# tensorboy/centerpose

Hardware: AMD Instinct MI355X
Metric: images/sec end-to-end (backbone+decode), DLA-34 512x512 (higher is better)
Workload: dtype f32

## Files before the change

centerpose_amd/csrc/plan_runtime.cpp:

```cpp
#include <cstdio>
#include <cstring>
#include <memory>
#include <string>
#include <vector>
#include "common.h"

extern "C" {
struct cp_conv_desc;
struct cp_dcn_desc;
int cp_abi_version(void);
int cp_conv2d_f32(const cp_conv_desc*, const float* const*, const float*, const float*, const float*, const float*, float*, void*);
int cp_conv3x3_winograd_f32(const cp_conv_desc*, const float*, const float*, const float*, const float*, const float*, float*, void*);
int cp_dcn_v2_f32(const cp_dcn_desc*, const float*, const float*, const float*, const float*, const float*, float*, void*);
int cp_conv3x3_winograd24_group_f32(const cp_conv_desc*, int, const float* const*, const float* const*, const float* const*, const float* const*,
                                    const float* const*, float* const*, void*);
int cp_conv2d_group_f32(const cp_conv_desc*, int, const float* const*, const float* const*, const float* const*, const float* const*,
                        const float* const*, float* const*, void*);
int cp_stem7x7_f32(const float*, const float*, const float*, const float*, float*, int, int, int, int, int, int, int, void*);
int cp_maxpool2d_nhwc_f32(const float*, int, float*, int, int, int, int, int, int, int, int, void*);
int cp_dw_deconv_add_nhwc_f32(const float*, int, const float*, const float*, int, float*, int, int, int, int, int, int, void*);
int cp_sum_up_nhwc_f32(int, const float* const*, const int*, const int*, float*, int, int, int, int, int, int, void*);
int cp_sum_up_group_nhwc_f32(int, const float* const*, const int*, float* const*, int, void*);
int cp_head3x3_1x1_f32(const cp_conv_desc*, const float*, const float*, const float*, const float*, const float*, const float*, float*, int,
                       int, int, void*);
int cp_dwconv2d_nhwc_f32(const float*, int, const float*, const float*, const float*, float*, int, int, int, int, int, int, int, int, int, void*);
int cp_global_avgpool_nhwc_f32(const float*, int, float*, int, int, int, int, void*);
int cp_scale_add_nhwc_f32(const float*, int, const float*, int, const float*, int, float*, int, int, int, int, int, void*);
int cp_shuffle_concat_nhwc_f32(const float*, int, const float*, int, float*, int, long long, int, int, void*);
int cp_multi_pose_decode_f32(const float*, const float*, const float*, const float*, const float*, const float*, int, int, int, int,
                             int, int, float*, float*, int*, void*);
int cp_splitk_reduce_f32(const float*, int, int, int, const float*, const float*, int, float*, int, int, void*);
int cp_sizeof_conv_desc(void);
int cp_sizeof_dcn_desc(void);
int cp_decode_topk_f32(const float*, const float*, int, int, int, int, int, int, float*, int*, void*);
int cp_decode_assign_f32(const float*, const float*, const float*, const float*, const float*, const int*, int, int, int, int, int, float*,
                         void*);
int cp_head_points_f32(const float*, int, const int*, const float*, const float*, const float*, const float*, float*, int, int, int, int, int,
                       int, int, void*);
int cp_flip_merge_pairs_f32(int, const float* const*, float* const*, const int*, int, int, int, int, const int*, void*);
int cp_head_points_pairs_f32(const float*, int, const int*, const int*, const float*, const float*, const float*, const float*, float*, int, int,
                             int, int, int, int, int, void*);
}

namespace {

enum { FN_CONV = 1, FN_WINO = 2, FN_DCN = 3, FN_STEM7 = 4, FN_POOL = 5, FN_UPADD = 6, FN_SUMUP = 7, FN_DWCONV = 8, FN_AVGPOOL = 9,
       FN_SCALEADD = 10, FN_SHUFFLE = 11, FN_HEAD = 12, FN_TOPK = 13, FN_ASSIGN = 14, FN_SPLITK = 15, FN_WINO24G = 16, FN_CONVG = 17, FN_SUMUPG = 18,
       FN_POINTS = 19, FN_FLIPPAIRS = 20, FN_POINTSPAIRS = 21 };
enum { REF_NULL = 0, REF_BUF = 1, REF_CONST = 2 };

struct Op {
    uint32_t fn = 0, out_index = 0, stream = 0;
    std::vector<unsigned char> desc;
    std::vector<float*> ptrs;
    std::vector<int> bufid;
    std::vector<int> ints;
};

struct Out { float* p; int shape[4]; int bufid; };

struct ConstPool {
    std::vector<float*> p;
    ~ConstPool() { for (float* q : p) if (q) (void)hipFree(q); }
};

}

struct cp_plan {
    int B = 0, H = 0, W = 0;
    std::vector<float*> bufs;
    std::vector<uint64_t> buf_numel;
// ... 36 lines not shown
    const int* I = o.ints.data();
    switch (o.fn) {
        case FN_CONV:
            return cp_conv2d_f32(reinterpret_cast<const cp_conv_desc*>(o.desc.data()), reinterpret_cast<const float* const*>(P.data()), P[4],
                                 P[5], P[6], P[7], P[8], s);
        case FN_WINO:
            return cp_conv3x3_winograd_f32(reinterpret_cast<const cp_conv_desc*>(o.desc.data()), P[0], P[1], P[2], P[3], P[4], P[5], s);
        case FN_DCN:
            return cp_dcn_v2_f32(reinterpret_cast<const cp_dcn_desc*>(o.desc.data()), P[0], P[1], P[2], P[3], P[4], P[5], s);
        case FN_WINO24G:
            return cp_conv3x3_winograd24_group_f32(reinterpret_cast<const cp_conv_desc*>(o.desc.data()), I[0], reinterpret_cast<const float* const*>(P.data()),
                                                   reinterpret_cast<const float* const*>(P.data() + 4), reinterpret_cast<const float* const*>(P.data() + 8),
                                                   reinterpret_cast<const float* const*>(P.data() + 12), reinterpret_cast<const float* const*>(P.data() + 16),
                                                   reinterpret_cast<float* const*>(P.data() + 20), s);
        case FN_CONVG:
            return cp_conv2d_group_f32(reinterpret_cast<const cp_conv_desc*>(o.desc.data()), I[0], reinterpret_cast<const float* const*>(P.data()),
                                       reinterpret_cast<const float* const*>(P.data() + 8), reinterpret_cast<const float* const*>(P.data() + 16),
                                       reinterpret_cast<const float* const*>(P.data() + 24), reinterpret_cast<const float* const*>(P.data() + 32),
                                       reinterpret_cast<float* const*>(P.data() + 40), s);
        case FN_STEM7:
            return cp_stem7x7_f32(P[0], P[1], P[2], P[3], P[4], I[0], I[1], I[2], I[3], I[4], I[5], I[6], s);
        case FN_POOL:
            return cp_maxpool2d_nhwc_f32(P[0], I[0], P[1], I[1], I[2], I[3], I[4], I[5], I[6], I[7], I[8], s);
        case FN_UPADD:
            return cp_dw_deconv_add_nhwc_f32(P[0], I[0], P[1], P[2], I[1], P[3], I[2], I[3], I[4], I[5], I[6], I[7], s);
        case FN_SUMUP:
            return cp_sum_up_nhwc_f32(I[0], reinterpret_cast<const float* const*>(P.data()), I + 1, I + 5, P[4], I[9], I[10], I[11], I[12],
                                      I[13], I[14], s);
        case FN_SUMUPG:
            return cp_sum_up_group_nhwc_f32(I[0], reinterpret_cast<const float* const*>(P.data()), I + 2, reinterpret_cast<float* const*>(P.data() + 16), I[1], s);
        case FN_HEAD:
            return cp_head3x3_1x1_f32(reinterpret_cast<const cp_conv_desc*>(o.desc.data()), P[0], P[1], P[2], P[3], P[4], P[5], P[6], I[0], I[1],
                                      I[2], s);
        case FN_DWCONV:
            return cp_dwconv2d_nhwc_f32(P[0], I[0], P[1], P[2], P[3], P[4], I[1], I[2], I[3], I[4], I[5], I[6], I[7], I[8], I[9], s);
        case FN_AVGPOOL:
            return cp_global_avgpool_nhwc_f32(P[0], I[0], P[1], I[1], I[2], I[3], I[4], s);
        case FN_SCALEADD:
            return cp_scale_add_nhwc_f32(P[0], I[0], P[1], I[1], P[2], I[2], P[3], I[3], I[4], I[5], I[6], I[7], s);
        case FN_SHUFFLE:
            return cp_shuffle_concat_nhwc_f32(P[0], I[0], P[1], I[1], P[2], I[2], (long long)I[3], I[4], I[5], s);
        case FN_SPLITK:
            return cp_splitk_reduce_f32(P[0], I[0], I[1], I[2], P[1], P[2], I[3], P[3], I[4], I[5], s);
        case FN_TOPK:
            return cp_decode_topk_f32(P[0], P[1], I[0], I[1], I[2], I[3], I[4], I[5], P[2], reinterpret_cast<int*>(P[3]), s);
        case FN_ASSIGN:
// ... 2 lines not shown
            return cp_head_points_f32(P[0], I[0], reinterpret_cast<const int*>(P[1]), P[2], P[3], P[4], P[5], P[6], I[1], I[2], I[3], I[4], I[5],
                                      I[6], I[7], s);
        case FN_FLIPPAIRS:
            return cp_flip_merge_pairs_f32(I[0], reinterpret_cast<const float* const*>(P.data()), reinterpret_cast<float* const*>(P.data() + 4), I + 5,
                                           I[1], I[2], I[3], I[4], reinterpret_cast<const int*>(P[8]), s);
        case FN_POINTSPAIRS:
            return cp_head_points_pairs_f32(P[0], I[0], reinterpret_cast<const int*>(P[1]), reinterpret_cast<const int*>(P[2]), P[3], P[4], P[5],
                                            P[6], P[7], I[1], I[2], I[3], I[4], I[5], I[6], I[7], s);
    }
    cp_set_error("plan: unknown launch function %u", o.fn);
    return 1;
}

bool arity_ok(const Op& o)
{
    switch (o.fn) {
        case FN_CONV: return o.ptrs.size() == 9 && (int)o.desc.size() == cp_sizeof_conv_desc();
        case FN_WINO: return o.ptrs.size() == 6 && (int)o.desc.size() == cp_sizeof_conv_desc();
        case FN_DCN: return o.ptrs.size() == 6 && (int)o.desc.size() == cp_sizeof_dcn_desc();
        case FN_WINO24G: return o.ptrs.size() == 25 && o.ints.size() == 1 && o.ints[0] >= 1 && o.ints[0] <= 4 && (int)o.desc.size() == 4 * cp_sizeof_conv_desc();
        case FN_CONVG: return o.ptrs.size() == 49 && o.ints.size() == 1 && o.ints[0] >= 1 && o.ints[0] <= 8 && (int)o.desc.size() == 8 * cp_sizeof_conv_desc();
        case FN_STEM7: return o.ptrs.size() == 5 && o.ints.size() == 7;
        case FN_POOL: return o.ptrs.size() == 2 && o.ints.size() == 9;
        case FN_UPADD: return o.ptrs.size() == 4 && o.ints.size() == 8;
        case FN_SUMUP: return o.ptrs.size() == 5 && o.ints.size() == 15;
        case FN_SUMUPG: return o.ptrs.size() == 21 && o.ints.size() == 58 && o.ints[0] >= 1 && o.ints[0] <= 4;
        case FN_HEAD: return o.ptrs.size() == 7 && o.ints.size() == 3 && (int)o.desc.size() == cp_sizeof_conv_desc();
        case FN_DWCONV: return o.ptrs.size() == 5 && o.ints.size() == 10;
        case FN_AVGPOOL: return o.ptrs.size() == 2 && o.ints.size() == 5;
        case FN_SCALEADD: return o.ptrs.size() == 4 && o.ints.size() == 8;
        case FN_SHUFFLE: return o.ptrs.size() == 3 && o.ints.size() == 6;
        case FN_SPLITK: return o.ptrs.size() == 4 && o.ints.size() == 6;
        case FN_TOPK: return o.ptrs.size() == 4 && o.ints.size() == 6;
        case FN_ASSIGN: return o.ptrs.size() == 7 && o.ints.size() == 5;
        case FN_POINTS: return o.ptrs.size() == 7 && o.ints.size() == 8;
        case FN_FLIPPAIRS: return o.ptrs.size() == 10 && o.ints.size() == 13 && o.ints[0] >= 1 && o.ints[0] <= 4;
        case FN_POINTSPAIRS: return o.ptrs.size() == 8 && o.ints.size() == 8;
    }
    return false;
}

int run_all(cp_plan* pl, hipStream_t s)
{
    for (const Op& o : pl->ops)
        if (int rc = run_op(o, s)) return rc;
    return 0;
// ... 440 lines not shown
```

centerpose_amd/engine.py:

```python
import os
import warnings
import weakref

import torch

from . import _lib, nets, ops
from .nets import Act


DECODE_TOPK = "decode.nms_topk"
SPARSE_HEADS = ("wh", "hps", "reg", "hp_offset")
FLIP_PEAKS = "flip.merge_peaks"
FLIP_IDX = ((1, 2), (3, 4), (5, 6), (7, 8), (9, 10), (11, 12), (13, 14), (15, 16))


def normalize_state_dict(sd, arch=None):
    out = {}
    for k, v in sd.items():
        if k.startswith("module") and not k.startswith("module_list"):
            k = k[7:]
        out[nets.internal_key(arch, k) if arch is not None else k] = v
    return out


# ... 23 lines not shown

    def give(self, slot):
        if self.reuse:
            self.free.append((self.clock(), slot))


class PlanBuilder(nets.Graph):
    def __init__(self, sd, B, device, sigmoid_heads=True, const_cache=None, dets_only=False):
        super().__init__()
        self.dets_only = dets_only
        self.points = None
        self.sd, self.B, self.dev = sd, B, device
        self.const_cache = const_cache if const_cache is not None else {}
        self.pool = BufferPool(device, lambda: len(self.launches))
        if isinstance(sigmoid_heads, bool):
            sigmoid_heads = ("hm", "hm_hp") if sigmoid_heads else ()
        self.sigmoid_heads = tuple(sigmoid_heads)
        self.launches = []
        self.winograd = os.environ.get("CP_WINOGRAD", "1") != "0"
        self.dcn_splitk = os.environ.get("CP_DCN_SPLITK", "1") != "0"
        self.wino_splitc = os.environ.get("CP_WINO_SPLITC", "1") != "0"
        self.conv_splitk = os.environ.get("CP_CONV_SPLITK", "1") != "0"
        self.fuse_heads = os.environ.get("CP_FUSE_HEADS", "1") != "0"
        self._pool_cache = {}
        self.outputs = None

    @property
    def bytes_alloc(self):
        return self.pool.bytes

    def buf(self, H, W, C, split=None):
        Cp = 2 * split[1] if split else ops.round_up(C, 16)
        slot = self.pool.take(self.B * H * W * Cp)
        act = Act(H, W, C, slot[: self.B * H * W * Cp].view(self.B, H, W, Cp), split)
        weakref.finalize(act, self.pool.give, slot)
        return act

    @staticmethod
    def cmap(a):
        if a.split:
            h, hp = a.split
            return list(range(h)) + list(range(hp, hp + h))
        return list(range(a.C))

    def expand_in(self, w, xs):
        if all(a.t.shape[3] == a.C and not a.split for a in xs):
            return w
# ... 54 lines not shown
        self.pool.give(ws)

    def add_conv3x3(self, name, flops, x, wp, u, sc, sh, out, cout, act, res=None, splitc=True):
        kind, wu = u if u is not None else ("conv", None)
        kw = dict(kh=3, kw=3, stride=1, pad=1, cout=cout, wino=wu, tile=ops.WINO24 if kind == "wino24" else 0)
        B, H, W, cin = x.shape
        S = ops.wino_ksplit(B, H, W, cin, cout) if (splitc and kind == "wino" and self.wino_splitc and res is None) else 1
        if S > 1:
            self.add_split(kind, name, ".splitc", flops, S, B * H * W, out.shape[3], lambda ones, zeros, ws: ops.conv2d_launch(
                [x], wp, ones, zeros, ws, ksplit=S, **kw), sc, sh, out, cout, act)
        else:
            self.add(kind, name, flops, ops.conv2d_launch([x], wp, sc, sh, out, act=act, res=res, **kw))

    def group_bufs(self, shapes):
        sizes = [self.B * H * W * Cp for H, W, _, Cp in shapes]
        slot = self.pool.take(sum(sizes))
        holder = Act(1, 1, 1, slot)
        weakref.finalize(holder, self.pool.give, slot)
        whole = slot[:sum(sizes)]
        return [Act(H, W, C, v.view(self.B, H, W, Cp), parent=holder) for (H, W, C, Cp), v in zip(shapes, whole.split(sizes))], whole

    def emit_conv(self, xs, conv, bn, bias, co, k, stride, pad, relu, res, stem):
        x = xs[0]
        Ho, Wo = (x.H + 2 * pad - k) // stride + 1, (x.W + 2 * pad - k) // stride + 1
        out = self.buf(Ho, Wo, co)
        if stem and k == 7 and pad == 3 and co in (16, 64) and res is None and bn and relu in (True, False):
            wp7 = ops.pack_stem7_weight(self.w(conv + ".weight"))
            sc7, sh7 = ops.fold_bn(co, self.bn(bn), self.w(conv + ".bias") if bias else None, self.dev)
            self.add("conv", conv, 2 * Ho * Wo * co * 3 * 49, ops.stem7x7_launch(xs[0].t, wp7, sc7, sh7, out.t, stride, relu))
            return out
        w = self.w(conv + ".weight")
        wp = ops.pack_conv_weight(w if stem else self.expand_in(w, xs), stem=stem)
        sc, sh = ops.fold_bn(co, self.bn(bn) if bn else None, self.w(conv + ".bias") if bias else None, self.dev)
        srcs = [a.t for a in xs]
        rt = res.t if res is not None else None
        ci = sum(a.C for a in xs)
        cip = ci if stem else sum(a.t.shape[3] for a in xs)
        u = None if stem else self.wino(wp, cip, co, conv, k, stride, pad, len(xs), hw=(x.H, x.W))
        flops = 2 * Ho * Wo * co * ci * k * k
        S = ops.conv_ksplit(ops.rule_batch(self.B) * Ho * Wo, wp.shape[0], wp.shape[1]) \
            if (self.conv_splitk and not stem and len(xs) == 1 and res is None and not (k == 3 and stride == 1 and pad == 1)) else 1
        if u is not None:
            self.add_conv3x3(conv, flops, srcs[0], wp, u, sc, sh, out.t, out.t.shape[3], self.act_code(relu), rt)
        elif S > 1:
            self.add_split("conv", conv, ".splitk", flops, S, self.B * Ho * Wo, wp.shape[0], lambda ones, zeros, ws: ops.conv2d_launch(
                srcs, wp, ones, zeros, ws, kh=k, kw=k, stride=stride, pad=pad, cout=ws.shape[2], ksplit=S),
# ... 31 lines not shown
            chunk = members[c0:c0 + ops.GROUP_MAX]
            if len(chunk) == 1:
                outs += super().emit_conv_batch(chunk)
                continue
            couts, whole = self.group_bufs([((x.H + 2 * pad - k) // stride + 1, (x.W + 2 * pad - k) // stride + 1, co, ops.round_up(co, 16))
                                            for x, _, _, co, k, stride, pad, _ in chunk])
            recs, flops = [], 0
            for (x, conv, bn, co, k, stride, pad, relu), out in zip(chunk, couts):
                wp = ops.pack_conv_weight(self.expand_in(self.w(conv + ".weight"), [x]))
                sc, sh = ops.fold_bn(co, self.bn(bn), None, self.dev)
                ldw = ops.round_up(wp.shape[0], 64)
                recs.append(dict(x=x.t, wp=ops.pad_rows(wp, ldw), scale=ops.pad_vec(sc, ldw), shift=ops.pad_vec(sh, ldw), out=out.t,
                                 cout=out.t.shape[3], k=k, stride=stride, pad=pad, act=self.act_code(relu)))
                flops += 2 * out.H * out.W * co * x.C * k * k
            self.add("conv", "group:" + chunk[0][1], flops, ops.conv2d_group_launch(recs, whole))
            outs += couts
        return outs

    def emit_maxpool(self, x, k, s, p):
        key = (id(x), k, s, p)
        hit = self._pool_cache.get(key)
        if hit is not None and hit[0]() is x and hit[1]() is not None:
            return hit[1]()
        out = self.buf((x.H + 2 * p - k) // s + 1, (x.W + 2 * p - k) // s + 1, x.C)
        self.add("pool", "maxpool%dx%d" % (k, k), 0, ops.maxpool2d_launch(x.t, out.t, k, s, p))
        self._pool_cache[key] = (weakref.ref(x), weakref.ref(out))
        return out

    def emit_dcn(self, x, conv, bn, co):
        om = self.buf(x.H, x.W, 32)
        wom = ops.pack_conv_weight(self.expand_in(self.w(conv + ".conv_offset_mask.weight"), [x]))
        som, hom = ops.fold_bn(27, None, self.w(conv + ".conv_offset_mask.bias"), self.dev)
        som[27:] = 0.0
        out = self.buf(x.H, x.W, co)
        wp = ops.pack_conv_weight(self.expand_in(self.w(conv + ".weight"), [x]))
        sc, sh = ops.fold_bn(co, self.bn(bn), self.w(conv + ".bias"), self.dev)
        uom = self.wino(wom, x.t.shape[3], 32, conv + ".conv_offset_mask", hw=(x.H, x.W))
        self.add_conv3x3(conv + ".conv_offset_mask", 2 * x.H * x.W * 27 * x.C * 9, x.t, wom, uom, som, hom, om.t, 32, ops.ACT_NONE)
        flops = 2 * x.H * x.W * co * x.C * 9
        S = ops.dcn_ksplit(ops.rule_batch(self.B) * x.H * x.W, wp.shape[0]) if self.dcn_splitk else 1
        if S > 1:
            self.add_split("dcn", conv, ".splitk", flops, S, self.B * x.H * x.W, wp.shape[0], lambda ones, zeros, ws: ops.dcn_v2_launch(
                x.t, om.t, wp, ones, zeros, ws, cout=ws.shape[2], om_sigmoid=True, ksplit=S), sc, sh, out.t, out.t.shape[3], ops.ACT_RELU)
        else:
            self.add("dcn", conv, flops,
                     ops.dcn_v2_launch(x.t, om.t, wp, sc, sh, out.t, cout=out.t.shape[3], om_sigmoid=True, act=ops.ACT_RELU))
        return out

    def emit_up_add(self, x, wname, f, add):
        out = self.buf(x.H * f, x.W * f, x.C)
# ... 439 lines not shown
        if g is None:
            g = torch.cuda.CUDAGraph()
            with torch.cuda.graph(g, capture_error_mode="thread_local"):
                self.run_eager()
            self.stream_of_launch = [0] * len(self.launches)
        self.graph = g

    def forward(self, images):
        if tuple(images.shape) != tuple(self.input.shape):
            raise ValueError("engine was planned for input %s, got %s" % (tuple(self.input.shape), tuple(images.shape)))
        if images.data_ptr() != self.input.data_ptr():
            self.input.copy_(images)
        if self.use_graph:
            if self.graph is None:
                self.capture()
            self.graph.replay()
        else:
            self.run_eager()
        return self.outputs

    __call__ = forward

    def launch_bytes(self, launches=None):
        grouped = ("cp_conv3x3_winograd24_group_f32", "cp_conv2d_group_f32", "cp_sum_up_group_nhwc_f32", "cp_flip_merge_pairs_f32")
        return [sum(4 * t.numel() for t in (launch.tensors[:-1] if launch.fn in grouped else launch.tensors) if t is not None)
                for _, _, _, launch in (self.launches if launches is None else launches)]

    def profile(self, iters=5):
        torch.cuda.synchronize(self.device)
        self.run_eager()
        nbytes = self.launch_bytes()
        recs = []
        for (kind, name, flops, launch), nb in zip(self.launches, nbytes):
            e0, e1 = torch.cuda.Event(enable_timing=True), torch.cuda.Event(enable_timing=True)
            e0.record()
            for _ in range(iters):
                launch.run()
            e1.record()
            e1.synchronize()
            recs.append(dict(kind=kind, name=name, fn=launch.fn, kernel=launch.kernel, flops=flops, bytes=nb, ms=e0.elapsed_time(e1) / iters))
        return recs

    def profile_in_sequence(self, iters=10):
        torch.cuda.synchronize(self.device)
        self.run_eager()
        n = len(self.launches)
        samples = [[] for _ in range(n)]
# ... 69 lines not shown
```

centerpose_amd/nets.py:

```python
from collections import OrderedDict

HEADS = (("hm", 1), ("wh", 2), ("hps", 34), ("reg", 2), ("hm_hp", 17), ("hp_offset", 2))
ARCH_HEAD = {"dla_34": (64, 256), "res_50": (256, 64), "hrnet": (32, 64), "mobilenetv3": (24, 256), "shufflenetV2": (256, 256),
             "resdcn_18": (64, 64), "resdcn_34": (64, 64), "resdcn_50": (64, 64), "resdcn_101": (64, 64)}
RESDCN_SPEC = {18: ("basic", [2, 2, 2, 2]), 34: ("basic", [3, 4, 6, 3]), 50: ("bottleneck", [3, 4, 6, 3]),
               101: ("bottleneck", [3, 4, 23, 3])}


class Act:
    __slots__ = ("H", "W", "C", "t", "split", "parent", "__weakref__")

    def __init__(self, H, W, C, t=None, split=None, parent=None):
        self.H, self.W, self.C, self.t, self.split = H, W, C, t, split
        self.parent = parent


class Graph:

    def __init__(self):
        self.spec = OrderedDict()
        self.flops = 0

    def p_conv(self, name, co, ci, k, bias=False, kw=None):
        self.spec[name + ".weight"] = (co, ci, k, kw or k)
        if bias:
            self.spec[name + ".bias"] = (co,)

    def p_bn(self, name, c):
        for s in ("weight", "bias", "running_mean", "running_var"):
            self.spec["%s.%s" % (name, s)] = (c,)
        self.spec[name + ".num_batches_tracked"] = ()

    def emit_conv(self, xs, conv, bn, bias, co, k, stride, pad, relu, res, stem):
        x = xs[0]
        return Act((x.H + 2 * pad - k) // stride + 1, (x.W + 2 * pad - k) // stride + 1, co)

    def emit_maxpool(self, x, k, s, p):
        return Act((x.H + 2 * p - k) // s + 1, (x.W + 2 * p - k) // s + 1, x.C)

    def emit_conv_group(self, members):
        return [self.emit_conv([x], conv, bn, False, co, 3, 1, 1, relu, res, False) for x, conv, bn, co, relu, res in members]

    def emit_conv_batch(self, members):
        return [self.emit_conv([x], conv, bn, False, co, k, stride, pad, relu, None, False) for x, conv, bn, co, k, stride, pad, relu in members]

    def emit_dcn(self, x, conv, bn, co):
        return Act(x.H, x.W, co)

    def emit_up_add(self, x, wname, f, add):
        return Act(x.H * f, x.W * f, x.C)

    def emit_deconv4(self, x, wname, bn, co):
        return Act(x.H * 2, x.W * 2, co)

    def emit_sum_up(self, xs, shifts, relu):
        return Act(xs[0].H, xs[0].W, xs[0].C)

    def emit_sum_up_batch(self, members, relu):
        return [self.emit_sum_up(xs, shifts, relu) for xs, shifts in members]

    def emit_head(self, feat, p, hc):
# ... 38 lines not shown
    def dwconv(self, x, name, bn, k, stride, act=None):
        self.spec[name + ".weight"] = (x.C, 1, k, k)
        self.p_bn(bn, x.C)
        out = self.emit_dwconv(x, name, bn, k, stride, act)
        self.flops += 2 * out.H * out.W * x.C * k * k
        return out

    def up_add(self, x, wname, f, add):
        self.spec[wname + ".weight"] = (x.C, 1, 2 * f, 2 * f)
        out = self.emit_up_add(x, wname, f, add)
        self.flops += 2 * out.H * out.W * x.C * 4
        return out

    def _dla_block(self, x, p, ci, co, stride, residual):
        h = self.conv(x, p + ".conv1", p + ".bn1", co, 3, stride, 1, relu=True)
        return self.conv(h, p + ".conv2", p + ".bn2", co, 3, 1, 1, relu=True, res=residual)

    def _dla_tree(self, x, p, levels, ci, co, stride, level_root, root_dim=0, children=None, top=True):
        children = [] if children is None else children
        if root_dim == 0:
            root_dim = 2 * co
        if level_root:
            root_dim += ci
        bottom = self.emit_maxpool(x, stride, stride, 0) if stride > 1 else x
        if ci != co:
            self.p_conv(p + ".project.0", co, ci, 1)
            self.p_bn(p + ".project.1", co)
        if level_root:
            children.append(bottom)
        if levels == 1:
            residual = bottom
            if ci != co:
                residual = self.emit_conv([bottom], p + ".project.0", p + ".project.1", False, co, 1, 1, 0, False, None, False)
                self.flops += 2 * residual.H * residual.W * co * ci
            x1 = self._dla_block(x, p + ".tree1", ci, co, stride, residual)
            x2 = self._dla_block(x1, p + ".tree2", co, co, 1, x1)
            return self.conv([x2, x1] + children, p + ".root.conv", p + ".root.bn", co, 1, relu=True)
        x1 = self._dla_tree(x, p + ".tree1", levels - 1, ci, co, stride, False)
        children.append(x1)
        return self._dla_tree(x1, p + ".tree2", levels - 1, co, co, 1, False, root_dim + co, children)

    def dla34(self, x, p="backbone_model"):
        ch, lv = [16, 32, 64, 128, 256, 512], [1, 1, 1, 2, 2, 1]
        b = p + ".base"
        y = []
        x = self.conv(x, b + ".base_layer.0", b + ".base_layer.1", 16, 7, 1, 3, relu=True, stem=True)
        x = self.conv(x, b + ".level0.0", b + ".level0.1", 16, 3, 1, 1, relu=True)
# ... 283 lines not shown
```

centerpose_amd/ops.py:

```python
import ctypes
import os

import torch

from . import _lib

ACT_NONE, ACT_RELU, ACT_SIGMOID, ACT_HSWISH, ACT_HSIGMOID = 0, 1, 2, 3, 4
BN_EPS = 1e-5


class ConvDesc(ctypes.Structure):
    _fields_ = [(n, ctypes.c_int) for n in ("nsrc",)] + [("srcC", ctypes.c_int * 4), ("srcLd", ctypes.c_int * 4)] + \
        [(n, ctypes.c_int) for n in ("B", "H", "W", "Ho", "Wo", "kh", "kw", "sy", "sx", "py", "px", "K", "ldw", "Cout",
                                     "resLd", "outLd", "outNCHW", "OH", "OW", "osy", "osx", "ooy", "oox", "act",
                                     "inNCHW", "tile", "nsub", "ksplit")]


class DcnDesc(ctypes.Structure):
    _fields_ = [(n, ctypes.c_int) for n in ("B", "H", "W", "C", "srcLd", "Ho", "Wo", "kh", "kw", "sy", "sx", "py", "px",
                                            "dily", "dilx", "K", "ldw", "Cout", "omLd", "omSigmoid", "outLd",
                                            "outNCHW", "act", "tile", "ksplit", "dg")]


def round_up(x, m):
# ... 31 lines not shown
        if self.kernel is None:
            self.kernel = _lib.lib().cp_last_kernel().decode()


def marshal(fn, desc, ptrs, ints):
    d = ctypes.byref(desc) if desc is not None else None
    if fn == "cp_conv2d_f32":
        srcs = (ctypes.c_void_p * 4)(*[p.value for p in ptrs[:4]])
        return [d, srcs] + ptrs[4:]
    if fn in ("cp_conv3x3_winograd_f32", "cp_dcn_v2_f32"):
        return [d] + ptrs
    if fn == "cp_conv3x3_winograd24_group_f32":
        arr = lambda k: (ctypes.c_void_p * 4)(*[p.value for p in ptrs[4 * k:4 * k + 4]])
        return [d, ints[0]] + [arr(k) for k in range(6)]
    if fn == "cp_conv2d_group_f32":
        arr = lambda k: (ctypes.c_void_p * 8)(*[p.value for p in ptrs[8 * k:8 * k + 8]])
        return [d, ints[0]] + [arr(k) for k in range(6)]
    if fn == "cp_head3x3_1x1_f32":
        return [d] + ptrs + ints
    if fn == "cp_stem7x7_f32":
        return ptrs + ints
    if fn == "cp_maxpool2d_nhwc_f32":
        return [ptrs[0], ints[0], ptrs[1]] + ints[1:]
    if fn == "cp_dw_deconv_add_nhwc_f32":
        return [ptrs[0], ints[0], ptrs[1], ptrs[2], ints[1], ptrs[3]] + ints[2:]
    if fn == "cp_sum_up_nhwc_f32":
        srcs = (ctypes.c_void_p * 4)(*[p.value for p in ptrs[:4]])
        lds = (ctypes.c_int * 4)(*ints[1:5])
        shs = (ctypes.c_int * 4)(*ints[5:9])
        return [ints[0], srcs, lds, shs, ptrs[4]] + ints[9:]
    if fn == "cp_sum_up_group_nhwc_f32":
        srcs = (ctypes.c_void_p * 16)(*[p.value for p in ptrs[:16]])
        outs = (ctypes.c_void_p * 4)(*[p.value for p in ptrs[16:20]])
        meta = (ctypes.c_int * 56)(*ints[2:58])
        return [ints[0], srcs, meta, outs, ints[1]]
    if fn == "cp_dwconv2d_nhwc_f32":
        return [ptrs[0], ints[0], ptrs[1], ptrs[2], ptrs[3], ptrs[4]] + ints[1:]
    if fn == "cp_global_avgpool_nhwc_f32":
        return [ptrs[0], ints[0], ptrs[1]] + ints[1:]
    if fn == "cp_scale_add_nhwc_f32":
        return [ptrs[0], ints[0], ptrs[1], ints[1], ptrs[2], ints[2], ptrs[3]] + ints[3:]
    if fn == "cp_shuffle_concat_nhwc_f32":
        return [ptrs[0], ints[0], ptrs[1], ints[1], ptrs[2], ints[2], ctypes.c_longlong(ints[3]), ints[4], ints[5]]
    if fn == "cp_splitk_reduce_f32":
        return [ptrs[0], ints[0], ints[1], ints[2], ptrs[1], ptrs[2], ints[3], ptrs[3], ints[4], ints[5]]
    if fn == "cp_decode_topk_f32":
        return ptrs[:2] + ints + ptrs[2:]
    if fn == "cp_decode_assign_f32":
        return ptrs[:6] + ints + [ptrs[6]]
    if fn == "cp_head_points_f32":
        return [ptrs[0], ints[0]] + ptrs[1:] + ints[1:]
    if fn == "cp_head_points_pairs_f32":
        return [ptrs[0], ints[0]] + ptrs[1:] + ints[1:]
    if fn == "cp_flip_merge_pairs_f32":
        ins = (ctypes.c_void_p * 4)(*[p.value for p in ptrs[:4]])
        outs = (ctypes.c_void_p * 4)(*[p.value for p in ptrs[4:8]])
        meta = (ctypes.c_int * 8)(*ints[5:13])
        return [ints[0], ins, outs, meta] + ints[1:5] + [ptrs[8]]
    raise ValueError("unknown launch function %r" % fn)


FN_IDS = {"cp_conv2d_f32": 1, "cp_conv3x3_winograd_f32": 2, "cp_dcn_v2_f32": 3, "cp_stem7x7_f32": 4,
          "cp_maxpool2d_nhwc_f32": 5, "cp_dw_deconv_add_nhwc_f32": 6, "cp_sum_up_nhwc_f32": 7, "cp_dwconv2d_nhwc_f32": 8,
          "cp_global_avgpool_nhwc_f32": 9, "cp_scale_add_nhwc_f32": 10, "cp_shuffle_concat_nhwc_f32": 11, "cp_head3x3_1x1_f32": 12,
          "cp_decode_topk_f32": 13, "cp_decode_assign_f32": 14, "cp_splitk_reduce_f32": 15, "cp_conv3x3_winograd24_group_f32": 16, "cp_conv2d_group_f32": 17,
          "cp_sum_up_group_nhwc_f32": 18, "cp_head_points_f32": 19,
          "cp_flip_merge_pairs_f32": 20, "cp_head_points_pairs_f32": 21}


def pad_rows(t, ldw):
    Co, K = t.shape
    if Co == ldw:
        return t.contiguous()
    out = torch.zeros((ldw, K), dtype=t.dtype, device=t.device)
    out[:Co] = t
    return out


def pad_vec(v, ldw, fill=0.0):
    out = torch.full((ldw,), fill, dtype=torch.float32, device=v.device)
    out[: v.numel()] = v
    return out


def ldw_for(cout):
    if cout <= 16:
        return 16
    if cout <= 32:
        return 32
    return round_up(cout, 64)
# ... 289 lines not shown
    return 1


def dcn_ksplit(M, ldw, taps=9):
    if ldw % 64 != 0 or taps < 3:
        return 1
    blocks = -(-M // 64) * (ldw // 64)
    return 3 if blocks < 512 else 1


def splitk_reduce_launch(ws, scale, shift, out, *, cout, act=ACT_NONE):
    S, M, ldw = ws.shape
    assert ws.is_contiguous() and out.shape[0] * out.shape[1] * out.shape[2] == M and scale.numel() >= ldw and shift.numel() >= ldw
    return Launch("cp_splitk_reduce_f32", None, [ws, scale, shift, out], [S, M, ldw, act, _ld(out), cout])


def maxpool2d_launch(x, out, k, s, p):
    B, H, W, C = x.shape
    return Launch("cp_maxpool2d_nhwc_f32", None, [x, out], [_ld(x), _ld(out), B, H, W, C, k, s, p])


def maxpool2d(x, out, k, s, p):
    maxpool2d_launch(x, out, k, s, p).run()
    return out


def pack_dw_deconv_weight(w):
    C, _, k, _ = w.shape
    return w.reshape(C, k * k).t().contiguous().float()


def dw_deconv_add_launch(x, wk, add, out, f):
    B, H, W, C = x.shape
    assert wk.is_contiguous()
    return Launch("cp_dw_deconv_add_nhwc_f32", None, [x, wk, add, out],
                  [_ld(x), _ld(add) if add is not None else 0, _ld(out), B, H, W, C, f])


def dw_deconv_add(x, wk, add, out, f):
    dw_deconv_add_launch(x, wk, add, out, f).run()
    return out


def pack_dw_weight(w):
    C, _, k, _ = w.shape
    return w.reshape(C, k * k).t().contiguous().float()
# ... 180 lines not shown
```

include/centerpose_hip.h:

```cpp
#ifndef CENTERPOSE_HIP_H
#define CENTERPOSE_HIP_H
#include <stddef.h>
#ifdef __cplusplus
extern "C" {
#endif

int cp_abi_version(void);
const char* cp_target_arch(void);
const char* cp_last_error(void);
const char* cp_last_kernel(void);

enum { CP_ACT_NONE = 0, CP_ACT_RELU = 1, CP_ACT_SIGMOID = 2,
       CP_ACT_HSWISH = 3, CP_ACT_HSIGMOID = 4 };

typedef struct cp_conv_desc {
    int nsrc;
    int srcC[4], srcLd[4];
    int B, H, W;
    int Ho, Wo;
    int kh, kw, sy, sx, py, px;
    int K, ldw;
    int Cout;
    int resLd, outLd;
    int outNCHW;
// ... 33 lines not shown
    int kh, kw, sy, sx, py, px, dily, dilx;
    int K, ldw, Cout;
    int omLd, omSigmoid;
    int outLd, outNCHW, act;
    int tile;
    int ksplit;
    int dg;
} cp_dcn_desc;
int cp_dcn_v2_f32(const cp_dcn_desc* d, const float* x, const float* om, const float* w, const float* scale,
                  const float* shift, float* out, void* stream);
int cp_dcn_pack_weights_f32(const float* w, const float* bias, int Co, int C, int kh, int kw, int dg, int Cp, int ldw, float* wp,
                            float* scale, float* shift, void* stream);
int cp_sizeof_conv_desc(void);
int cp_sizeof_dcn_desc(void);

int cp_splitk_reduce_f32(const float* ws, int splits, int M, int ldw, const float* scale, const float* shift, int act, float* out,
                         int outLd, int Cout, void* stream);

int cp_stem7x7_f32(const float* x, const float* w, const float* scale, const float* shift, float* out, int B, int H, int W,
                   int Cout, int stride, int outLd, int relu, void* stream);

int cp_maxpool2d_nhwc_f32(const float* in, int inLd, float* out, int outLd, int B, int H, int W, int C, int k, int s, int p,
                          void* stream);
int cp_dw_deconv_add_nhwc_f32(const float* in, int inLd, const float* w, const float* add, int addLd, float* out, int outLd,
                              int B, int H, int W, int C, int f, void* stream);
int cp_sum_up_nhwc_f32(int n, const float* const* src, const int* ld, const int* shift, float* out, int outLd, int B, int H,
                       int W, int C, int relu, void* stream);
int cp_sum_up_group_nhwc_f32(int n, const float* const* src, const int* meta, float* const* out, int relu, void* stream);
int cp_dwconv2d_nhwc_f32(const float* in, int inLd, const float* w, const float* scale, const float* shift, float* out, int outLd,
                         int B, int H, int W, int C, int k, int s, int p, int act, void* stream);
int cp_global_avgpool_nhwc_f32(const float* in, int inLd, float* out, int outLd, int B, int HW, int C, void* stream);
int cp_scale_add_nhwc_f32(const float* x, int xLd, const float* se, int seLd, const float* add, int addLd, float* out, int outLd,
                          int B, int H, int W, int C, void* stream);
int cp_shuffle_concat_nhwc_f32(const float* x1, int ld1, const float* x2, int ld2, float* out, int outLd, long long npix, int h, int hp,
                               void* stream);
int cp_nchw_to_nhwc_f32(const float* in, float* out, int B, int C, int H, int W, int outLd, int cOff, void* stream);
int cp_nhwc_to_nchw_f32(const float* in, int inLd, int cOff, float* out, int B, int C, int H, int W, void* stream);
int cp_fill_f32(float* p, float v, long long n, void* stream);
int cp_flip_merge_f32(const float* in, float* out, int C, int H, int W, int mode, const int* perm, void* stream);
int cp_flip_merge_pairs_f32(int n, const float* const* in, float* const* out, const int* meta, int N, int H, int W, int J,
                            const int* perm, void* stream);

int cp_resize_u8(const unsigned char* src, int H, int W, unsigned char* dst, int NH, int NW, void* stream);
int cp_preprocess_u8_f32(const unsigned char* img, int H, int W, const double* M, float* out, int OH, int OW, const float* mean,
                         const float* std_, int flip, void* stream);
int cp_transform_dets_f32(const float* dets, float* out, const double* trans, int B, int K, int J, float scale, void* stream);
// ... 71 lines not shown
```

Before: 2224.

## Fuse 2x2 maxpool downsample with the following 1x1 projection conv in DLA trees

Adds a HIP kernel that performs the 2x2 stride-2 max pool and the 1x1 project conv plus folded BN in one launch, using MFMA f32 on the pooled tile held in LDS. The pooled tensor is still written out by the first column tile so the residual path can use it. The engine records the projected output so the later project conv emission is skipped. This removes a separate pool launch and a re-read of the pooled activations, at the cost of a new GEMM path whose tiling may be less efficient than the general conv kernel.

```diff
diff --git a/centerpose_amd/csrc/plan_runtime.cpp b/centerpose_amd/csrc/plan_runtime.cpp
--- a/centerpose_amd/csrc/plan_runtime.cpp
+++ b/centerpose_amd/csrc/plan_runtime.cpp
@@ -18,6 +18,7 @@
                         const float* const*, float* const*, void*);
 int cp_stem7x7_f32(const float*, const float*, const float*, const float*, float*, int, int, int, int, int, int, int, void*);
 int cp_maxpool2d_nhwc_f32(const float*, int, float*, int, int, int, int, int, int, int, int, void*);
+int cp_pool_project_f32(const float*, int, const float*, const float*, const float*, float*, int, float*, int, int, int, int, int, int, int, void*);
 int cp_dw_deconv_add_nhwc_f32(const float*, int, const float*, const float*, int, float*, int, int, int, int, int, int, void*);
 int cp_sum_up_nhwc_f32(int, const float* const*, const int*, const int*, float*, int, int, int, int, int, int, void*);
 int cp_sum_up_group_nhwc_f32(int, const float* const*, const int*, float* const*, int, void*);
@@ -46,7 +47,7 @@
 
 enum { FN_CONV = 1, FN_WINO = 2, FN_DCN = 3, FN_STEM7 = 4, FN_POOL = 5, FN_UPADD = 6, FN_SUMUP = 7, FN_DWCONV = 8, FN_AVGPOOL = 9,
        FN_SCALEADD = 10, FN_SHUFFLE = 11, FN_HEAD = 12, FN_TOPK = 13, FN_ASSIGN = 14, FN_SPLITK = 15, FN_WINO24G = 16, FN_CONVG = 17, FN_SUMUPG = 18,
-       FN_POINTS = 19, FN_FLIPPAIRS = 20, FN_POINTSPAIRS = 21 };
+       FN_POINTS = 19, FN_FLIPPAIRS = 20, FN_POINTSPAIRS = 21, FN_POOLPROJ = 22 };
 enum { REF_NULL = 0, REF_BUF = 1, REF_CONST = 2 };
 
 struct Op {
@@ -129,6 +130,8 @@
             return cp_stem7x7_f32(P[0], P[1], P[2], P[3], P[4], I[0], I[1], I[2], I[3], I[4], I[5], I[6], s);
         case FN_POOL:
             return cp_maxpool2d_nhwc_f32(P[0], I[0], P[1], I[1], I[2], I[3], I[4], I[5], I[6], I[7], I[8], s);
+        case FN_POOLPROJ:
+            return cp_pool_project_f32(P[0], I[0], P[1], P[2], P[3], P[4], I[1], P[5], I[2], I[3], I[4], I[5], I[6], I[7], I[8], s);
         case FN_UPADD:
             return cp_dw_deconv_add_nhwc_f32(P[0], I[0], P[1], P[2], I[1], P[3], I[2], I[3], I[4], I[5], I[6], I[7], s);
         case FN_SUMUP:
@@ -177,6 +180,7 @@
         case FN_CONVG: return o.ptrs.size() == 49 && o.ints.size() == 1 && o.ints[0] >= 1 && o.ints[0] <= 8 && (int)o.desc.size() == 8 * cp_sizeof_conv_desc();
         case FN_STEM7: return o.ptrs.size() == 5 && o.ints.size() == 7;
         case FN_POOL: return o.ptrs.size() == 2 && o.ints.size() == 9;
+        case FN_POOLPROJ: return o.ptrs.size() == 7 && o.ints.size() == 9;
         case FN_UPADD: return o.ptrs.size() == 4 && o.ints.size() == 8;
         case FN_SUMUP: return o.ptrs.size() == 5 && o.ints.size() == 15;
         case FN_SUMUPG: return o.ptrs.size() == 21 && o.ints.size() == 58 && o.ints[0] >= 1 && o.ints[0] <= 4;
diff --git a/centerpose_amd/csrc/pool_project.hip b/centerpose_amd/csrc/pool_project.hip
--- /dev/null
+++ b/centerpose_amd/csrc/pool_project.hip
@@ -0,0 +1,182 @@
+#include <cmath>
+#include "igemm.h"
+
+struct PoolProjArgs {
+    const float* x;
+    const float* w;
+    const float* scale;
+    const float* shift;
+    float* pooled;
+    float* out;
+    int xLd, poolLd, outLd;
+    int H, W, Ho, Wo, M;
+    int ldw, Cout;
+};
+
+template <int KK>
+struct PpTile {
+    static constexpr int BM = 64, BN = 64;
+    static constexpr int LDK = KK + 4;
+    static constexpr int CH = KK < 64 ? KK : 64;
+    static constexpr int NCH = KK / CH;
+    static constexpr int Q = CH / 4;
+    static constexpr int SLOTS = BM * Q / IG_THREADS;
+    static constexpr int ROWS = IG_THREADS / Q;
+    static constexpr int R_SLOTS = BM * BN / 4 / IG_THREADS;
+    static constexpr int LDC = BN + 4;
+    static constexpr int MAIN_BYTES = (BM + BN) * LDK * 4, EPI_BYTES = BM * LDC * 4;
+    static constexpr int SMEM = MAIN_BYTES > EPI_BYTES ? MAIN_BYTES : EPI_BYTES;
+    static_assert(KK % IG_BK == 0 && KK % CH == 0 && (BM * Q) % IG_THREADS == 0 && BM == BN, "tile");
+};
+
+__device__ __forceinline__ float4 pp_max4(float4 m, float4 v)
+{
+    return make_float4(fmaxf(m.x, v.x), fmaxf(m.y, v.y), fmaxf(m.z, v.z), fmaxf(m.w, v.w));
+}
+
+template <int KK, int OCC>
+__global__ __launch_bounds__(IG_THREADS, OCC) void pool_project_kernel(const PoolProjArgs a)
+{
+    using T = PpTile<KK>;
+    constexpr int BM = T::BM, BN = T::BN, LDK = T::LDK, Q = T::Q, CH = T::CH;
+    extern __shared__ __attribute__((aligned(16))) float smem[];
+    float* As = smem;
+    float* Bs = smem + BM * LDK;
+    const int tid = threadIdx.x, lane = tid & 63, wid = tid >> 6;
+    const int NT = a.ldw / BN;
+    const int tile = ig_xcd_remap(blockIdx.x, gridDim.x);
+    const int nt = tile % NT, mt = tile / NT;
+    const int m0 = mt * BM, n0 = nt * BN;
+    const int wm0 = (wid >> 1) * 32, wn0 = (wid & 1) * 32;
+
+    const int c4 = tid % Q, r0 = tid / Q;
+    const int HoWo = a.Ho * a.Wo, rowLd = a.W * a.xLd;
+    unsigned xoff[T::SLOTS];
+    bool mok[T::SLOTS];
+#pragma unroll
+    for (int s = 0; s < T::SLOTS; ++s) {
+        const int m = m0 + r0 + s * T::ROWS;
+        mok[s] = m < a.M;
+        const int mm = mok[s] ? m : 0;
+        const int b = mm / HoWo, p = mm - b * HoWo, oy = p / a.Wo, ox = p - oy * a.Wo;
+        xoff[s] = (unsigned)((b * a.H + 2 * oy) * a.W + 2 * ox) * (unsigned)a.xLd + (unsigned)c4 * 4u;
+    }
+    const bool wr = a.pooled != nullptr && nt == 0;
+    const int rc4 = tid & 15, n = n0 + rc4 * 4;
+    const bool nok = n < a.Cout;
+    float4 sc = make_float4(1.f, 1.f, 1.f, 1.f), sh = make_float4(0.f, 0.f, 0.f, 0.f);
+    if (nok) { sc = ig_ldg4(a.scale + n); sh = ig_ldg4(a.shift + n); }
+
+#pragma unroll
+    for (int c = 0; c < T::NCH; ++c) {
+        float4 v[T::SLOTS][4], br[T::SLOTS];
+#pragma unroll
+        for (int s = 0; s < T::SLOTS; ++s) {
+            const float* p = a.x + c * CH + xoff[s];
+            v[s][0] = ig_ldg4(p);
+            v[s][1] = ig_ldg4(p + a.xLd);
+            v[s][2] = ig_ldg4(p + rowLd);
+            v[s][3] = ig_ldg4(p + rowLd + a.xLd);
+        }
+#pragma unroll
+        for (int s = 0; s < T::SLOTS; ++s)
+            br[s] = ig_ldg4(a.w + (size_t)(n0 + r0 + s * T::ROWS) * KK + c * CH + c4 * 4);
+#pragma unroll
+        for (int s = 0; s < T::SLOTS; ++s) {
+            const int row = r0 + s * T::ROWS;
+            float4 m = make_float4(-INFINITY, -INFINITY, -INFINITY, -INFINITY);
+            m = pp_max4(pp_max4(pp_max4(pp_max4(m, v[s][0]), v[s][1]), v[s][2]), v[s][3]);
+            *reinterpret_cast<float4*>(As + row * LDK + c * CH + c4 * 4) = m;
+            if (wr && mok[s]) *reinterpret_cast<float4*>(a.pooled + (size_t)(m0 + row) * a.poolLd + c * CH + c4 * 4) = m;
+        }
+#pragma unroll
+        for (int s = 0; s < T::SLOTS; ++s)
+            *reinterpret_cast<float4*>(Bs + (r0 + s * T::ROWS) * LDK + c * CH + c4 * 4) = br[s];
+    }
+    __syncthreads();
+
+    f32x16 acc;
+#pragma unroll
+    for (int r = 0; r < 16; ++r) acc[r] = 0.f;
+    const int g = lane >> 5, il = lane & 31;
+    const float* ap = As + (wm0 + il) * LDK + g * 4;
+    const float* bp = Bs + (wn0 + il) * LDK + g * 4;
+#pragma unroll
+    for (int ks = 0; ks < KK / IG_BK; ++ks) {
+        float4 af[2], bf[2];
+#pragma unroll
+        for (int h = 0; h < 2; ++h) {
+            af[h] = *reinterpret_cast<const float4*>(ap + ks * IG_BK + h * 8);
+            bf[h] = *reinterpret_cast<const float4*>(bp + ks * IG_BK + h * 8);
+        }
+#pragma unroll
+        for (int h = 0; h < 2; ++h) {
+            acc = __builtin_amdgcn_mfma_f32_32x32x2f32(af[h].x, bf[h].x, acc, 0, 0, 0);
+            acc = __builtin_amdgcn_mfma_f32_32x32x2f32(af[h].y, bf[h].y, acc, 0, 0, 0);
+            acc = __builtin_amdgcn_mfma_f32_32x32x2f32(af[h].z, bf[h].z, acc, 0, 0, 0);
+            acc = __builtin_amdgcn_mfma_f32_32x32x2f32(af[h].w, bf[h].w, acc, 0, 0, 0);
+        }
+    }
+
+    float* Cs = smem;
+    constexpr int LDC = T::LDC;
+    __syncthreads();
+#pragma unroll
+    for (int r = 0; r < 16; ++r) Cs[(wm0 + ig_row<32>(r, lane)) * LDC + wn0 + il] = acc[r];
+    __syncthreads();
+#pragma unroll
+    for (int s = 0; s < T::R_SLOTS; ++s) {
+        const int row = (tid >> 4) + s * 16, m = m0 + row;
+        if (m < a.M && nok) {
+            const float4 v = *reinterpret_cast<const float4*>(Cs + row * LDC + rc4 * 4);
+            *reinterpret_cast<float4*>(a.out + (size_t)m * a.outLd + n) = cp_scale_shift4(v, sc, sh);
+        }
+    }
+}
+
+template <int KK, int OCC>
+static int launch_pp(const PoolProjArgs& a, hipStream_t s)
+{
+    using T = PpTile<KK>;
+    auto kern = pool_project_kernel<KK, OCC>;
+    static CpLdsGuard guard;
+    if (T::SMEM > 64 * 1024) {
+        const hipError_t e = guard.ensure((const void*)kern, T::SMEM);
+        if (e != hipSuccess) { cp_set_error("pool_project: cannot reserve %d B LDS: %s", T::SMEM, hipGetErrorString(e)); return 2; }
+    }
+    const long long grid = (long long)cp_cdiv(a.M, T::BM) * (a.ldw / T::BN);
+    CP_CHECK_ARG(grid < (1ll << 31), "pool_project: grid %lld too large", grid);
+    hipLaunchKernelGGL(kern, dim3((unsigned)grid), dim3(IG_THREADS), T::SMEM, s, a);
+    cp_note_kernel("pool_project_kernel<%d>", KK);
+    return 0;
+}
+
+extern "C" int cp_pool_project_f32(const float* x, int xLd, const float* w, const float* scale, const float* shift, float* pooled,
+                                   int poolLd, float* out, int outLd, int B, int H, int W, int K, int ldw, int Cout, void* stream)
+{
+    CP_CHECK_ARG(x && w && scale && shift && out, "pool_project: null pointer");
+    CP_CHECK_ARG(B > 0 && H >= 2 && W >= 2, "pool_project: bad problem size B=%d H=%d W=%d", B, H, W);
+    CP_CHECK_ARG(xLd % 4 == 0 && xLd >= K && outLd % 4 == 0 && Cout % 4 == 0 && Cout > 0 && outLd >= Cout && ldw % 64 == 0 && ldw >= Cout,
+                 "pool_project: xLd=%d outLd=%d Cout=%d ldw=%d (ld, Cout multiples of 4; ldw a multiple of 64)", xLd, outLd, Cout, ldw);
+    CP_CHECK_ARG(!pooled || (poolLd % 4 == 0 && poolLd >= K), "pool_project: poolLd=%d (K=%d)", poolLd, K);
+    CP_CHECK_ARG((((size_t)x | (size_t)w | (size_t)scale | (size_t)shift | (size_t)pooled | (size_t)out) & 15) == 0,
+                 "pool_project: tensors must be 16-byte aligned");
+    CP_CHECK_ARG((long long)B * H * W * xLd * 4 < (1ll << 32), "pool_project: source exceeds 32-bit byte offsets");
+    PoolProjArgs a;
+    a.x = x; a.w = w; a.scale = scale; a.shift = shift; a.pooled = pooled; a.out = out;
+    a.xLd = xLd; a.poolLd = poolLd; a.outLd = outLd;
+    a.H = H; a.W = W; a.Ho = H / 2; a.Wo = W / 2; a.M = B * a.Ho * a.Wo;
+    a.ldw = ldw; a.Cout = Cout;
+    hipStream_t s = (hipStream_t)stream;
+    int rc = 0;
+    switch (K) {
+        case 32: rc = launch_pp<32, 4>(a, s); break;
+        case 64: rc = launch_pp<64, 4>(a, s); break;
+        case 128: rc = launch_pp<128, 2>(a, s); break;
+        case 256: rc = launch_pp<256, 1>(a, s); break;
+        default: CP_CHECK_ARG(false, "pool_project: K=%d (32, 64, 128 or 256)", K);
+    }
+    if (rc) return rc;
+    CP_CHECK_LAUNCH("pool_project_kernel");
+    return 0;
+}
diff --git a/centerpose_amd/engine.py b/centerpose_amd/engine.py
--- a/centerpose_amd/engine.py
+++ b/centerpose_amd/engine.py
@@ -69,7 +69,10 @@
         self.wino_splitc = os.environ.get("CP_WINO_SPLITC", "1") != "0"
         self.conv_splitk = os.environ.get("CP_CONV_SPLITK", "1") != "0"
         self.fuse_heads = os.environ.get("CP_FUSE_HEADS", "1") != "0"
+        self.pool_project = os.environ.get("CP_POOL_PROJECT", "1") != "0"
         self._pool_cache = {}
+        self._project = None
+        self._projected = {}
         self.outputs = None
 
     @property
@@ -170,6 +173,9 @@
 
     def emit_conv(self, xs, conv, bn, bias, co, k, stride, pad, relu, res, stem):
         x = xs[0]
+        hit = self._projected.pop((id(x), conv), None)
+        if hit is not None and hit[0] is x:
+            return hit[1]
         Ho, Wo = (x.H + 2 * pad - k) // stride + 1, (x.W + 2 * pad - k) // stride + 1
         out = self.buf(Ho, Wo, co)
         if stem and k == 7 and pad == 3 and co in (16, 64) and res is None and bn and relu in (True, False):
@@ -247,10 +253,26 @@
         hit = self._pool_cache.get(key)
         if hit is not None and hit[0]() is x and hit[1]() is not None:
             return hit[1]()
-        out = self.buf((x.H + 2 * p - k) // s + 1, (x.W + 2 * p - k) // s + 1, x.C)
-        self.add("pool", "maxpool%dx%d" % (k, k), 0, ops.maxpool2d_launch(x.t, out.t, k, s, p))
+        Ho, Wo = (x.H + 2 * p - k) // s + 1, (x.W + 2 * p - k) // s + 1
+        if self._project is not None and (k, s, p) == (2, 2, 0) and not x.split and ops.pool_project_wanted(x.t.shape[3], self._project[2]):
+            conv, bn, co = self._project
+            (out, proj), whole = self.group_bufs([(Ho, Wo, x.C, x.t.shape[3]), (Ho, Wo, co, ops.round_up(co, 16))])
+            wp = ops.pack_conv_weight(self.expand_in(self.w(conv + ".weight"), [out]))
+            sc, sh = ops.fold_bn(co, self.bn(bn), None, self.dev)
+            self.add("conv", "pool+" + conv, 2 * Ho * Wo * co * x.C, ops.pool_project_launch(x.t, wp, sc, sh, out.t, proj.t, whole))
+            self._projected[(id(out), conv)] = (out, proj)
+        else:
+            out = self.buf(Ho, Wo, x.C)
+            self.add("pool", "maxpool%dx%d" % (k, k), 0, ops.maxpool2d_launch(x.t, out.t, k, s, p))
         self._pool_cache[key] = (weakref.ref(x), weakref.ref(out))
         return out
+
+    def downsample(self, x, stride, proj, co):
+        self._project = (proj + ".0", proj + ".1", co) if proj and self.pool_project else None
+        try:
+            return self.emit_maxpool(x, stride, stride, 0)
+        finally:
+            self._project = None
 
     def emit_dcn(self, x, conv, bn, co):
         om = self.buf(x.H, x.W, 32)
@@ -736,7 +758,7 @@
     __call__ = forward
 
     def launch_bytes(self, launches=None):
-        grouped = ("cp_conv3x3_winograd24_group_f32", "cp_conv2d_group_f32", "cp_sum_up_group_nhwc_f32", "cp_flip_merge_pairs_f32")
+        grouped = ("cp_conv3x3_winograd24_group_f32", "cp_conv2d_group_f32", "cp_sum_up_group_nhwc_f32", "cp_flip_merge_pairs_f32", "cp_pool_project_f32")
         return [sum(4 * t.numel() for t in (launch.tensors[:-1] if launch.fn in grouped else launch.tensors) if t is not None)
                 for _, _, _, launch in (self.launches if launches is None else launches)]
 
diff --git a/centerpose_amd/nets.py b/centerpose_amd/nets.py
--- a/centerpose_amd/nets.py
+++ b/centerpose_amd/nets.py
@@ -37,6 +37,9 @@
 
     def emit_maxpool(self, x, k, s, p):
         return Act((x.H + 2 * p - k) // s + 1, (x.W + 2 * p - k) // s + 1, x.C)
+
+    def downsample(self, x, stride, proj, co):
+        return self.emit_maxpool(x, stride, stride, 0)
 
     def emit_conv_group(self, members):
         return [self.emit_conv([x], conv, bn, False, co, 3, 1, 1, relu, res, False) for x, conv, bn, co, relu, res in members]
@@ -121,7 +124,7 @@
             root_dim = 2 * co
         if level_root:
             root_dim += ci
-        bottom = self.emit_maxpool(x, stride, stride, 0) if stride > 1 else x
+        bottom = self.downsample(x, stride, p + ".tree1" * (levels - 1) + ".project" if ci != co else None, co) if stride > 1 else x
         if ci != co:
             self.p_conv(p + ".project.0", co, ci, 1)
             self.p_bn(p + ".project.1", co)
diff --git a/centerpose_amd/ops.py b/centerpose_amd/ops.py
--- a/centerpose_amd/ops.py
+++ b/centerpose_amd/ops.py
@@ -77,6 +77,8 @@
         return ptrs + ints
     if fn == "cp_maxpool2d_nhwc_f32":
         return [ptrs[0], ints[0], ptrs[1]] + ints[1:]
+    if fn == "cp_pool_project_f32":
+        return [ptrs[0], ints[0], ptrs[1], ptrs[2], ptrs[3], ptrs[4], ints[1], ptrs[5], ints[2]] + ints[3:]
     if fn == "cp_dw_deconv_add_nhwc_f32":
         return [ptrs[0], ints[0], ptrs[1], ptrs[2], ints[1], ptrs[3]] + ints[2:]
     if fn == "cp_sum_up_nhwc_f32":
@@ -120,7 +122,7 @@
           "cp_global_avgpool_nhwc_f32": 9, "cp_scale_add_nhwc_f32": 10, "cp_shuffle_concat_nhwc_f32": 11, "cp_head3x3_1x1_f32": 12,
           "cp_decode_topk_f32": 13, "cp_decode_assign_f32": 14, "cp_splitk_reduce_f32": 15, "cp_conv3x3_winograd24_group_f32": 16, "cp_conv2d_group_f32": 17,
           "cp_sum_up_group_nhwc_f32": 18, "cp_head_points_f32": 19,
-          "cp_flip_merge_pairs_f32": 20, "cp_head_points_pairs_f32": 21}
+          "cp_flip_merge_pairs_f32": 20, "cp_head_points_pairs_f32": 21, "cp_pool_project_f32": 22}
 
 
 def pad_rows(t, ldw):
@@ -456,6 +458,27 @@
 
 def maxpool2d(x, out, k, s, p):
     maxpool2d_launch(x, out, k, s, p).run()
+
+
+POOL_PROJECT_K = (32, 64, 128, 256)
+
+
+def pool_project_wanted(K, cout):
+    return K in (32, 64, 128) and ldw_for(cout) % 64 == 0
+
+
+def pool_project_launch(x, wp, scale, shift, pooled, out, whole=None):
+    B, H, W, K = x.shape
+    assert K in POOL_PROJECT_K and tuple(wp.shape[1:]) == (K,) and wp.shape[0] % 64 == 0 and wp.is_contiguous()
+    assert tuple(out.shape[:3]) == (B, H // 2, W // 2) and out.shape[3] <= wp.shape[0] and scale.numel() == shift.numel() == wp.shape[0]
+    assert pooled is None or (tuple(pooled.shape[:3]) == (B, H // 2, W // 2) and pooled.shape[3] >= K)
+    if whole is None:
+        assert pooled is None
+        whole = out
+    for t in (pooled, out):
+        assert t is None or t.untyped_storage().data_ptr() == whole.untyped_storage().data_ptr()
+    return Launch("cp_pool_project_f32", None, [x, wp, scale, shift, pooled, out, whole],
+                  [_ld(x), _ld(pooled) if pooled is not None else 0, _ld(out), B, H, W, K, wp.shape[0], out.shape[3]])
     return out
 
 
diff --git a/include/centerpose_hip.h b/include/centerpose_hip.h
--- a/include/centerpose_hip.h
+++ b/include/centerpose_hip.h
@@ -79,6 +79,8 @@
 
 int cp_maxpool2d_nhwc_f32(const float* in, int inLd, float* out, int outLd, int B, int H, int W, int C, int k, int s, int p,
                           void* stream);
+int cp_pool_project_f32(const float* x, int xLd, const float* w, const float* scale, const float* shift, float* pooled, int poolLd,
+                        float* out, int outLd, int B, int H, int W, int K, int ldw, int Cout, void* stream);
 int cp_dw_deconv_add_nhwc_f32(const float* in, int inLd, const float* w, const float* add, int addLd, float* out, int outLd,
                               int B, int H, int W, int C, int f, void* stream);
 int cp_sum_up_nhwc_f32(int n, const float* const* src, const int* ld, const int* shift, float* out, int outLd, int B, int H,
```

Result: no change. 2232 (median of 4 runs) (+0.4%).
